# XuyangBai/D3Feat

Measured on AMD Instinct MI355X. Metric: fragments/sec (30k-pt clouds), higher is better.
Workload: dtype f32; 1 GPU; SURVEY §8d config #2: synthetic 3DMatch room fragment, 300k raw pts -> grid subsample 0.03 m (~29k pts per cloud) -> self-pair -> 5-level pyramid -> full KPFCNN forward (random-init weights (reference initialiser, seed 42), 14.1M params)...; points_per_cloud=29369, fragments_per_gpu=2141, parallelism=fragment-dp1, fragments_per_replay=12, engine_fallbacks=0, engine_isolated_replays=0

## Files before the change

### d3feat_amd/csrc/grid_subsample.hip

```cpp
#include <cstdlib>
#include "prims.h"
#include "radix_sort.h"

#define GS_EMPTY 0xFFFFFFFFFFFFFFFFull
#define GS_KEYBITS 56
#define GS_KEYMASK ((1ull << GS_KEYBITS) - 1ull)
#define GS_MAX_PROBE 4096

__constant__ unsigned long long D3F_CHAIN_DEV[D3F_NCHAIN] = {
    13ull, 29ull, 59ull, 127ull, 257ull, 541ull, 1109ull, 2357ull, 5087ull, 10273ull, 20753ull, 42043ull, 85229ull,
    172933ull, 351061ull, 712697ull, 1447153ull, 2938679ull, 5967347ull, 12117689ull, 24607243ull, 49969847ull,
    101473717ull, 206062531ull, 418451333ull, 849749479ull, 1725587117ull, 3504151727ull};

struct GsElem {
    float org[3];
    int pad0;
    unsigned long long NX, NY, NZ;
    long long bbase;
};

#include "gs_order.h"

__device__ __forceinline__ float gs_axis(unsigned mn, unsigned mx, float dl, float inv, float& org) {
    org = __fmul_rn(floorf(__fmul_rn(d3f_ord2f(mn), inv)), dl);
    return fmaxf(floorf(__fdiv_rn(__fsub_rn(d3f_ord2f(mx), org), dl)), 0.f);
}
__device__ __forceinline__ int gs_cell(const float* __restrict__ p, float ox, float oy, float oz, float dl, float& cx, float& cy,
                                       float& cz) {
    const float fx = floorf(__fdiv_rn(__fsub_rn(p[0], ox), dl));
    const float fy = floorf(__fdiv_rn(__fsub_rn(p[1], oy), dl));
    const float fz = floorf(__fdiv_rn(__fsub_rn(p[2], oz), dl));
    cx = fmaxf(fx, 0.f);
    cy = fmaxf(fy, 0.f);
    cz = fmaxf(fz, 0.f);
    return (fx < 0.f || fy < 0.f || fz < 0.f) ? D3F_ST_NEG_CELL : 0;
}

__device__ __forceinline__ float gs_inv_count(int c) { return (float)(1.0 / (double)c); }

__device__ __forceinline__ unsigned long long gs_mix(unsigned long long x) {
    x ^= x >> 33; x *= 0xff51afd7ed558ccdull; x ^= x >> 33; x *= 0xc4ceb9fe1a85ec53ull; x ^= x >> 33;
    return x;
}

__device__ __forceinline__ int gs_bits(unsigned long long x) {
    int b = 0;
    while (x) { ++b; x >>= 1; }
    return b;
}
__device__ __forceinline__ void gs_prep(const unsigned* __restrict__ bbox, const int* __restrict__ offs, int B, float dl,
                                        GsElem* __restrict__ el, int* __restrict__ status, RsMeta* __restrict__ smeta,
                                        int n_cap) {
    __shared__ unsigned long long sCells[256];
    const int b = threadIdx.x;
    unsigned long long cells = 0ull;
    if (b < B) {
        GsElem e;
        e.pad0 = 0;
        const int len = offs[b + 1] - offs[b];
        if (len <= 0) {
            atomicOr(&status[1], D3F_ST_EMPTY_ELEMENT);
            e.org[0] = e.org[1] = e.org[2] = 0.f;
            e.NX = e.NY = e.NZ = 1;
        } else {
            const float inv = __fdiv_rn(1.0f, dl);
            unsigned long long dims[3];
#pragma unroll
            for (int d = 0; d < 3; ++d) {
                const unsigned mn = __hip_atomic_load(&bbox[b * 6 + d], __ATOMIC_RELAXED, __HIP_MEMORY_SCOPE_AGENT);
                const unsigned mx = __hip_atomic_load(&bbox[b * 6 + 3 + d], __ATOMIC_RELAXED, __HIP_MEMORY_SCOPE_AGENT);
                dims[d] = (unsigned long long)gs_axis(mn, mx, dl, inv, e.org[d]) + 1ull;
            }
            e.NX = dims[0]; e.NY = dims[1]; e.NZ = dims[2];
        }
        long long base = 0;
        for (int j = 0; j < b; ++j) {
            long long l = offs[j + 1] - offs[j];
            unsigned long long nb = D3F_CHAIN_DEV[D3F_NCHAIN - 1];
            for (int c = 0; c < D3F_NCHAIN; ++c)
                if ((long long)D3F_CHAIN_DEV[c] >= l) { nb = D3F_CHAIN_DEV[c]; break; }
            base += (long long)nb;
        }
        e.bbase = base;
        el[b] = e;
        const double c = (double)e.NX * (double)e.NY * (double)e.NZ;
        cells = c >= 1.8e19 ? 0xFFFFFFFFFFFFFFFFull : e.NX * e.NY * e.NZ;
    }
    if (!smeta) return;
    sCells[threadIdx.x] = cells;
    __syncthreads();
    if (threadIdx.x == 0) {
        unsigned long long mx = 1ull;
        for (int j = 0; j < B; ++j) mx = sCells[j] > mx ? sCells[j] : mx;
        int kb = gs_bits(mx - 1ull);
        if (kb < 1) kb = 1;
        const int eb = gs_bits((unsigned long long)(B - 1));
        RsMeta m;
        m.n = min(offs[B], n_cap);
        m.kb = kb;
        m.bits = kb + eb;
        if (m.bits > 32) {
            atomicOr(&status[1], D3F_ST_KEY_WIDTH);
            m.n = 0;
            m.bits = 8;
        }
        m.npass = (m.bits + 7) / 8;
        *smeta = m;
    }
}
struct GsPrepEpi {
    const unsigned* bbox; const int* offs; int B; float dl; GsElem* el; int* status; RsMeta* smeta; int n_cap;
    __device__ __forceinline__ void operator()() const { gs_prep(bbox, offs, B, dl, el, status, smeta, n_cap); }
};

__global__ void __launch_bounds__(256) gs_begin_boxed_kernel(const int* __restrict__ lens, int B, int* __restrict__ offs,
                                                             const unsigned* __restrict__ bbox, unsigned* __restrict__ counters,
                                                             int ncounters, D3fFill f0, D3fFill fmeta, float dl, GsElem* __restrict__ el,
                                                             int* __restrict__ status, RsMeta* __restrict__ smeta, int n_cap) {
    const size_t tid = (size_t)blockIdx.x * blockDim.x + threadIdx.x, stride = (size_t)gridDim.x * blockDim.x;
    d3f_fill_words(f0, tid, stride);
    if (blockIdx.x != 0) return;
    if (threadIdx.x == 0) {
        int s = 0;
        for (int b = 0; b < B; ++b) { offs[b] = s; s += lens[b]; }
        offs[B] = s;
    }
    for (int i = threadIdx.x; i < ncounters; i += blockDim.x) counters[i] = 0u;
    for (int i = threadIdx.x; i < (int)fmeta.n; i += blockDim.x) fmeta.p[i] = fmeta.v;
    asm volatile("s_waitcnt vmcnt(0)" ::: "memory");
    __syncthreads();
    gs_prep(bbox, offs, B, dl, el, status, smeta, n_cap);
}

__global__ void __launch_bounds__(256) gs_insert_kernel(const float* __restrict__ pts, int N, const int* __restrict__ offs,
                                                        int B, float dl, const GsElem* __restrict__ el,
                                                        unsigned long long* __restrict__ tkey, unsigned* __restrict__ tfirst,
                                                        unsigned long long capmask, int* __restrict__ slot,
                                                        int* __restrict__ status) {
    const int i = blockIdx.x * blockDim.x + threadIdx.x;
    if (i >= min(N, offs[B])) return;
    const int b = d3f_find_elem(offs, B, i);
    const GsElem e = el[b];
    float cx, cy, cz;
    int st = gs_cell(pts + 3 * (size_t)i, e.org[0], e.org[1], e.org[2], dl, cx, cy, cz);
    const unsigned long long ix = (unsigned long long)cx, iy = (unsigned long long)cy, iz = (unsigned long long)cz;
    const unsigned long long key = ix + e.NX * iy + e.NX * e.NY * iz;
    if (key > GS_KEYMASK) st |= D3F_ST_KEY_RANGE;
    if (st) atomicOr(&status[1], st);
    const unsigned long long word = ((unsigned long long)b << GS_KEYBITS) | (key & GS_KEYMASK);
    unsigned long long h = gs_mix(word) & capmask;
    bool placed = false;
    for (int probe = 0; probe < GS_MAX_PROBE; ++probe) {
        unsigned long long prev = atomicCAS(&tkey[h], GS_EMPTY, word);
        if (prev == GS_EMPTY || prev == word) { placed = true; break; }
        h = (h + 1) & capmask;
    }
    if (!placed) atomicOr(&status[1], D3F_ST_OUT_OVERFLOW);
    atomicMin(&tfirst[h], (unsigned)i);
    slot[i] = (int)h;
}

struct GsMarkIn {
    const int* n_dev; const int* slot; const unsigned* tfirst;
    __device__ __forceinline__ int operator()(int i) const { return (i < *n_dev && tfirst[slot[i]] == (unsigned)i) ? 1 : 0; }
// ... 262 lines not shown
    }
    __syncthreads();
    const int w = threadIdx.x >> 6, lane = threadIdx.x & 63;
    const int base = tile * RS_TILE + w * RS_WAVE_ITEMS + lane;
    const int wlo = tile * RS_TILE + w * RS_WAVE_ITEMS, whi = min(wlo + RS_WAVE_ITEMS, n) - 1;
    int b0 = 0;
    while (b0 + 1 < B && wlo >= sOffs[b0 + 1]) ++b0;
    const bool one_cloud = (b0 + 1 >= B) || whi < sOffs[b0 + 1];
    unsigned key[RS_ROUNDS], vm = 0u;
    int st = 0;
#pragma unroll
    for (int r = 0; r < RS_ROUNDS; ++r) {
        const int i = base + r * 64;
        key[r] = 0u;
        if (i < n) {
            int b = b0;
            if (!one_cloud)
                while (b + 1 < B && i >= sOffs[b + 1]) ++b;
            const float ox = sEl[b].org[0], oy = sEl[b].org[1], oz = sEl[b].org[2];
            const unsigned NX = (unsigned)sEl[b].NX, NY = (unsigned)sEl[b].NY;
            const float* __restrict__ P = sBase[b];
            float cx, cy, cz;
            st |= gs_cell(P + 3 * (size_t)i, ox, oy, oz, dl, cx, cy, cz);
            const unsigned ix = (unsigned)cx, iy = (unsigned)cy, iz = (unsigned)cz;
            const unsigned k = ix + NX * (iy + NY * iz);
            key[r] = (kb < 32 ? ((unsigned)b << kb) : 0u) | (kb < 32 ? (k & ((1u << kb) - 1u)) : k);
            skey[i] = key[r];
            vm |= 1u << r;
        }
    }
    if (st) atomicOr(&status[1], st);
    rs_tile_histogram(key, vm, 0, sHist, hist + (size_t)tile * 256);
}

__global__ void __launch_bounds__(256) gs_heads_kernel(int N, const RsMeta* __restrict__ smeta, const unsigned* __restrict__ key0,
                                                       const unsigned* __restrict__ key1, const unsigned* __restrict__ val0,
                                                       const unsigned* __restrict__ val1, unsigned* __restrict__ fbits) {
    const int j = blockIdx.x * blockDim.x + threadIdx.x;
    if (j >= min(N, smeta->n)) return;
    const unsigned* __restrict__ ks = (smeta->npass & 1) ? key1 : key0;
    const unsigned* __restrict__ vs = (smeta->npass & 1) ? val1 : val0;
    const unsigned k = ks[j];
    if (j == 0 || ks[j - 1] != k) {
        const unsigned i = vs[j];
        atomicOr(&fbits[i >> 5], 1u << (i & 31u));
    }
}
struct GsBitsIn {
    const unsigned* fbits;
    __device__ __forceinline__ int operator()(int w) const { return __popc(fbits[w]); }
};
__global__ void __launch_bounds__(256) gs_runs_kernel(int N, const RsMeta* __restrict__ smeta, const unsigned* __restrict__ key0,
                                                      const unsigned* __restrict__ key1, const unsigned* __restrict__ val0,
                                                      const unsigned* __restrict__ val1, GsRankBits rank,
                                                      const float* __restrict__ pts, const float* const* __restrict__ ptrs,
                                                      const int* __restrict__ offs, unsigned long long* __restrict__ vkey,
                                                      float* __restrict__ bary) {
    __shared__ float sx[256], sy[256], sz[256];
    __shared__ unsigned sk[256];
    const int n = min(N, smeta->n);
    const int j0 = blockIdx.x * 256;
    if (j0 >= n) return;
    const int t = threadIdx.x, j = j0 + t;
    const unsigned* __restrict__ ks = (smeta->npass & 1) ? key1 : key0;
    const unsigned* __restrict__ vs = (smeta->npass & 1) ? val1 : val0;
    unsigned k = 0u, pi = 0u, kprev = 0u;
    float px = 0.f, py = 0.f, pz = 0.f;
    if (j < n) {
        k = ks[j];
        pi = vs[j];
        kprev = j > 0 ? ks[j - 1] : 0u;
        if (ptrs) {
            const int b = smeta->kb < 32 ? (int)(k >> smeta->kb) : 0;
            pts = ptrs[b] - 3 * (size_t)offs[b];
        }
        px = pts[3 * (size_t)pi + 0]; py = pts[3 * (size_t)pi + 1]; pz = pts[3 * (size_t)pi + 2];
    }
    sx[t] = px; sy[t] = py; sz[t] = pz;
    sk[t] = k;
    __syncthreads();
    if (j >= n || (j != 0 && kprev == k)) return;
    const int v = rank((int)pi);
    float ax = px, ay = py, az = pz;
    int c = 1;
    const int lim = min(256, n - j0);
    while (t + c < lim && sk[t + c] == k) {
        ax = __fadd_rn(ax, sx[t + c]);
        ay = __fadd_rn(ay, sy[t + c]);
        az = __fadd_rn(az, sz[t + c]);
        ++c;
    }
    if (t + c == 256) {
        while (j + c < n && ks[j + c] == k) {
            const size_t q = vs[j + c];
            ax = __fadd_rn(ax, pts[3 * q + 0]);
            ay = __fadd_rn(ay, pts[3 * q + 1]);
            az = __fadd_rn(az, pts[3 * q + 2]);
            ++c;
        }
    }
    const float sc = gs_inv_count(c);
    vkey[v] = (unsigned long long)(smeta->kb < 32 ? (k & ((1u << smeta->kb) - 1u)) : k);
    bary[3 * (size_t)v + 0] = __fmul_rn(ax, sc);
    bary[3 * (size_t)v + 1] = __fmul_rn(ay, sc);
    bary[3 * (size_t)v + 2] = __fmul_rn(az, sc);
}
template <bool BOX>
__global__ void __launch_bounds__(BOX ? 1024 : 256) gs_emit_kernel(int* __restrict__ status, const int* __restrict__ moffs, int B,
                                                      const int* __restrict__ vpos, const float* __restrict__ bary,
                                                      float* __restrict__ out_p, int out_cap, unsigned* __restrict__ bbox_out) {
    const int v = blockIdx.x * blockDim.x + threadIdx.x;
    bool ok = v < status[0] && !(status[1] & (D3F_ST_OUT_OVERFLOW | D3F_ST_KEY_WIDTH));
    int b = -1;
    float x = 0.f, y = 0.f, z = 0.f;
    if (ok) {
        b = d3f_find_elem(moffs, B, v);
        const size_t dest = (size_t)moffs[b] + (size_t)vpos[v];
        if (dest >= (size_t)out_cap) {
            atomicOr(&status[1], D3F_ST_OUT_OVERFLOW);
            ok = false;
        } else {
            x = bary[3 * (size_t)v + 0]; y = bary[3 * (size_t)v + 1]; z = bary[3 * (size_t)v + 2];
            out_p[3 * dest + 0] = x;
            out_p[3 * dest + 1] = y;
            out_p[3 * dest + 2] = z;
        }
// ... 49 lines not shown
    const size_t dest = (size_t)moffs[b] + (size_t)vpos[v];
    for (int l = 0; l < ldim; ++l) atomicMax(&out_c[dest * ldim + l], cls[(size_t)i * ldim + l]);
}

struct GsLayout {
    size_t cap;
    long long bucket_total;
};
static GsLayout gs_layout(int N, int B, int keys = -1) {
    GsLayout L;
    L.cap = 64;
    const size_t nk = (size_t)((keys > 0 && keys < N) ? keys : (N > 0 ? N : 1));
    while (L.cap < (size_t)2 * nk) L.cap <<= 1;
    L.bucket_total = (long long)(2.24 * (double)N) + 16ll * B + 64;
    return L;
}

extern "C" size_t d3f_grid_subsample_workspace_bytes(int N, int B, int fdim, int ldim) {
    (void)fdim; (void)ldim;
    if (N < 0 || B < 1) return 0;
    GsLayout L = gs_layout(N, B);
    size_t n = (size_t)(N > 0 ? N : 1);
    size_t bytes = 0;
    bytes += d3f_align((B + 1) * sizeof(int)) * 2 + d3f_align((B + 2) * sizeof(int));
    bytes += d3f_align(B * 6 * sizeof(unsigned));
    bytes += d3f_align(B * sizeof(GsElem));
    bytes += d3f_align(L.cap * sizeof(unsigned long long));
    bytes += d3f_align(L.cap * sizeof(int));
    bytes += d3f_align(n * sizeof(unsigned long long));
    bytes += 16 * d3f_align(n * sizeof(int));
    bytes += 6 * d3f_align((size_t)L.bucket_total * sizeof(int));
    bytes += d3f_align((n / GS_TILE + B + 8) * sizeof(int));
    bytes += 2 * d3f_align(d3f_scan_base_ints(N) * sizeof(int)) + d3f_align((4 + D3F_NCHAIN * (size_t)B) * sizeof(unsigned));
    bytes += d3f_align(rs_hist_words(N) * sizeof(unsigned)) + d3f_align((n / 32 + 2) * sizeof(unsigned)) +
             d3f_align(3 * n * sizeof(float)) + d3f_align(sizeof(RsMeta));
    bytes += d3f_align(7 * (size_t)B * (n < 16384 ? n : 16384) * sizeof(float)) + 256 + 2 * d3f_align(B * sizeof(int));
    return bytes + 4096;
}

template <int T, int R>
static int gs_small_launch(const GsSmallArgs& A, float* sub_points, int* sub_lens_dev, int* status_dev, hipStream_t stream) {
    static std::atomic<unsigned long long> lds_done{0ull};
    const void* const fns[] = {(const void*)gs_small_kernel<T, R>};
    if (d3f_opt_in_lds(lds_done, fns, (int)gss_lds_bytes<T, R>(GSS_NB_MAX)) != D3F_OK) return D3F_ERR_HIP;
    gs_small_kernel<T, R><<<A.B, T, gss_lds_bytes<T, R>(A.nbmax), stream>>>(A);
    D3F_LAUNCH_CHECK();
    gs_small_pack_kernel<<<d3f_cdiv(A.out_cap, 256), 256, 0, stream>>>(A, sub_points, sub_lens_dev, status_dev);
    D3F_LAUNCH_CHECK();
    return D3F_OK;
}
static int gs_run_small(const float* points, int N, const int* lens_dev, int B, float dl, float* sub_points, int M_cap, int elem_cap,
                        int pc, int* sub_lens_dev, int* status_dev, void* workspace, size_t workspace_bytes, hipStream_t stream,
                        unsigned* bbox_out = nullptr) {
    if (elem_cap <= 0 || elem_cap > M_cap) elem_cap = M_cap;
    if (elem_cap > pc) elem_cap = pc;
    D3fArena ar(workspace, workspace_bytes);
    GsSmallArgs A;
    A.stage = ar.take<float>(3 * (size_t)B * (size_t)elem_cap);
    A.recs = ar.take<float>(4 * (size_t)B * (size_t)elem_cap);
    A.mcount = ar.take<int>(B);
    A.cflags = ar.take<int>(B);
    if (!ar.ok) return D3F_ERR_WORKSPACE;
    A.bbox_out = bbox_out;
    A.pts = points; A.lens = lens_dev; A.B = B; A.dl = dl; A.elem_cap = elem_cap; A.pc = pc; A.out_cap = M_cap;
    A.nbmax = GSS_NB_MAX;
    for (int j = 0; j < D3F_NCHAIN; ++j)
        if ((long long)D3F_CHAIN_HOST[j] >= (long long)elem_cap) { A.nbmax = (int)D3F_CHAIN_HOST[j]; break; }
    if (A.nbmax > GSS_NB_MAX) A.nbmax = GSS_NB_MAX;
// ... 8 lines not shown
struct GsCall {
    const float* points; int N; const int* lens_dev; int B; float dl;
    const float* features; int fdim; const int* classes; int ldim;
    float* sub_points; int M_cap; float* sub_features; int* sub_classes; int* sub_lens_dev;
    int* status_host;
    int* status_dev;
    hipStream_t stream;
    const float* const* ptrs;
    const unsigned* bbox_in;
    unsigned* bbox_out;
};

struct GsWork {
    GsLayout L;
    int *offs, *moffs;
    unsigned* bbox;
    GsElem* el;
    int ncounters;
    unsigned* counters;
    unsigned long long* tkey;
    unsigned* tfirst;
    int* vhead;
    int* meta;
    int* vcnt;
    unsigned long long* vkey;
    int *slot, *vscan, *pvid, *pnext, *vstart, *sorted;
    GsOrderArgs A;
    int* vbase;
    int* sbase;
    unsigned* rs_hist;
    unsigned* fbits;
    float* bary;
    RsMeta* smeta;

    bool carve(void* workspace, size_t workspace_bytes, int N, int B, int keys) {
        L = gs_layout(N, B, keys);
        D3fArena ar(workspace, workspace_bytes);
        const size_t n = (size_t)N;
        offs = ar.take<int>(B + 1);
        moffs = ar.take<int>(B + 1);
        bbox = ar.take<unsigned>(B * 6);
        el = ar.take<GsElem>(B);
        ncounters = 4 + D3F_NCHAIN * B;
        counters = ar.take<unsigned>(ncounters);
        tkey = ar.take<unsigned long long>(L.cap);
        tfirst = ar.take<unsigned>(L.cap);
        vhead = ar.take<int>(n);
        meta = ar.take<int>(B + 2);
        vcnt = ar.take<int>(n);
        vkey = ar.take<unsigned long long>(n);
        slot = ar.take<int>(n);
        vscan = ar.take<int>(n);
        pvid = ar.take<int>(n);
        pnext = ar.take<int>(n);
        vstart = ar.take<int>(n);
        sorted = ar.take<int>(n);
        A.vpos = ar.take<int>(n);
        A.P[0] = ar.take<int>(n);
        A.P[1] = ar.take<int>(n);
        A.nx[0] = ar.take<int>(n);
        A.nx[1] = ar.take<int>(n);
        A.cd = ar.take<int>(n);
        A.bkt[0] = ar.take<int>(n);
        A.bkt[1] = ar.take<int>(n);
        for (int k = 0; k < 2; ++k) {
            A.bf[k] = ar.take<int>((size_t)L.bucket_total);
            A.bc[k] = ar.take<int>((size_t)L.bucket_total);
            A.bh[k] = ar.take<int>((size_t)L.bucket_total);
        }
        A.tsum = ar.take<int>(n / GS_TILE + B + 8);
        vbase = ar.take<int>(d3f_scan_base_ints(N));
        sbase = ar.take<int>(d3f_scan_base_ints(N));
        rs_hist = ar.take<unsigned>(rs_hist_words(N));
        fbits = ar.take<unsigned>(n / 32 + 2);
        bary = ar.take<float>(3 * n);
        smeta = ar.take<RsMeta>(1);
        A.vkey = vkey; A.moffs = moffs; A.offs = offs; A.el = el;
        return ar.ok;
    }
};

static int gs_order_launch(const GsWork& W, int B, int maxM, hipStream_t stream) {
    gs_order_small_kernel<<<B, GS_SMALL_T, 0, stream>>>(W.A);
    for (int j = GS_SMALL_LAST + 1; j < D3F_NCHAIN && (long long)D3F_CHAIN_HOST[j - 1] < (long long)maxM; ++j) {
        const long long nbj = (long long)D3F_CHAIN_HOST[j];
        const int hi = (int)((long long)maxM < nbj ? (long long)maxM : nbj);
        const bool more = j + 1 < D3F_NCHAIN && nbj < (long long)maxM;
        const long long nbn = more ? (long long)D3F_CHAIN_HOST[j + 1] : 0;
        const int hin = more ? (int)((long long)maxM < nbn ? (long long)maxM : nbn) : hi;
        dim3 g(d3f_cdiv(hi, 256), B), gt(d3f_cdiv(hi, GS_TILE), B), gp(d3f_cdiv(hin > hi ? hin : hi, 256), B);
        if (j == GS_SMALL_LAST + 1) gs_order_insert_kernel<<<g, 256, 0, stream>>>(W.A, j);
        gs_order_scan_tiles_kernel<<<gt, 256, 0, stream>>>(W.A, j, B, W.counters + 4 + j * B);
        gs_order_place_kernel<<<gp, 256, 0, stream>>>(W.A, j);
    }
    D3F_LAUNCH_CHECK();
    return D3F_OK;
}

static int gs_run_sort(const GsCall& C, const GsWork& W, int elem_cap) {
    const int N = C.N, B = C.B;
    const size_t n = (size_t)N;
    hipStream_t stream = C.stream;
    int rc;
    const D3fFill none{nullptr, 0ull, 0u};
    const D3fFill fill_bits{W.fbits, (unsigned long long)(n / 32 + 2), 0u};
    const D3fFill fill_meta{(unsigned*)W.meta, (unsigned long long)(B + 2), 0u};
    if (C.bbox_in) {
        long long blocks = (long long)(fill_bits.n / 4 / 256) + 1;
        if (blocks > 1024) blocks = 1024;
        gs_begin_boxed_kernel<<<(int)blocks, 256, 0, stream>>>(C.lens_dev, B, W.offs, C.bbox_in, W.counters, W.ncounters, fill_bits,
                                                               fill_meta, C.dl, W.el, W.meta, W.smeta, N);
        D3F_LAUNCH_CHECK();
    } else {
        if ((rc = d3f_begin_launch(C.lens_dev, B, W.offs, W.bbox, W.counters, W.ncounters, fill_bits, fill_meta, none, none,
                                   stream)) != D3F_OK)
            return rc;
        GsPrepEpi prep{W.bbox, W.offs, B, C.dl, W.el, W.meta, W.smeta, N};
        if ((rc = d3f_bbox_launch_t(C.points, W.offs, B, N, W.bbox, W.counters, prep, stream, C.ptrs)) != D3F_OK) return rc;
    }
    const int nblk = d3f_cdiv(N, 256);
    unsigned *key0 = (unsigned*)W.slot, *key1 = (unsigned*)W.pnext, *val0 = (unsigned*)W.pvid, *val1 = (unsigned*)W.sorted;
    gs_sortkey_kernel<<<rs_tiles(N), RS_THREADS, 0, stream>>>(C.points, C.ptrs, W.offs, B, C.dl, W.el, W.smeta, key0, W.rs_hist,
                                                              W.meta);
    D3F_LAUNCH_CHECK();
    if ((rc = rs_sort_launch(W.smeta, N, key0, key1, val0, val1, W.rs_hist, stream)) != D3F_OK) return rc;
    gs_heads_kernel<<<nblk, 256, 0, stream>>>(N, W.smeta, key0, key1, val0, val1, W.fbits);
    D3F_LAUNCH_CHECK();
    const GsRankBits rank{W.fbits, W.vscan, W.vbase};
    GsMoffsEpi<GsRankBits> mepi{W.offs, B, rank, W.meta, W.moffs, C.sub_lens_dev, C.status_dev, C.M_cap, elem_cap};
    if ((rc = d3f_scan_fold_launch(GsBitsIn{W.fbits}, N / 32 + 1, nullptr, W.vscan, W.vbase, W.counters + 1, mepi, stream)) != D3F_OK)
        return rc;
    gs_runs_kernel<<<nblk, 256, 0, stream>>>(N, W.smeta, key0, key1, val0, val1, rank, C.points, C.ptrs, W.offs, W.vkey, W.bary);
    D3F_LAUNCH_CHECK();
    const int M = N < C.M_cap ? N : C.M_cap;
    if ((rc = gs_order_launch(W, B, elem_cap, stream)) != D3F_OK) return rc;
    if (C.bbox_out)
        gs_emit_kernel<true><<<d3f_cdiv(M, 1024), 1024, 0, stream>>>(W.meta, W.moffs, B, W.A.vpos, W.bary, C.sub_points, C.M_cap,
                                                                     C.bbox_out);
    else
        gs_emit_kernel<false><<<d3f_cdiv(M, 256), 256, 0, stream>>>(W.meta, W.moffs, B, W.A.vpos, W.bary, C.sub_points, C.M_cap,
                                                                    nullptr);
    D3F_LAUNCH_CHECK();
    return D3F_OK;
}

static int gs_run_hash(const GsCall& C, const GsWork& W, int elem_cap) {
    const int N = C.N, B = C.B;
    const size_t n = (size_t)N;
    const bool async = C.status_dev != nullptr;
    hipStream_t stream = C.stream;
    int rc;
    const D3fFill none{nullptr, 0ull, 0u};
    const unsigned long long ones_words = (unsigned long long)((char*)(W.vhead + n) - (char*)W.tkey) / 4ull;
    const unsigned long long zero_words = (unsigned long long)((char*)(W.vcnt + n) - (char*)W.meta) / 4ull;
    if ((rc = d3f_begin_launch(C.lens_dev, B, W.offs, W.bbox, W.counters, W.ncounters, D3fFill{(unsigned*)W.tkey, ones_words, 0xFFFFFFFFu},
                               D3fFill{(unsigned*)W.meta, zero_words, 0u}, none, none, stream)) != D3F_OK)
        return rc;
    GsPrepEpi prep{W.bbox, W.offs, B, C.dl, W.el, W.meta, nullptr, N};
    if ((rc = d3f_bbox_launch_t(C.points, W.offs, B, N, W.bbox, W.counters, prep, stream, C.ptrs)) != D3F_OK) return rc;
    const int nblk = d3f_cdiv(N, 256);
    GsMoffsEpi<GsRankScan> mepi{W.offs, B, GsRankScan{W.vscan, W.vbase}, W.meta, W.moffs, C.sub_lens_dev, C.status_dev, C.M_cap,
                                async ? elem_cap : 0x7fffffff};
    gs_insert_kernel<<<nblk, 256, 0, stream>>>(C.points, N, W.offs, B, C.dl, W.el, W.tkey, W.tfirst, (unsigned long long)W.L.cap - 1ull,
                                               W.slot, W.meta);
    D3F_LAUNCH_CHECK();
    if ((rc = d3f_scan_fold_launch(GsMarkIn{W.offs + B, W.slot, W.tfirst}, N, W.offs + B, W.vscan, W.vbase, W.counters + 1, mepi,
                                   stream)) != D3F_OK)
        return rc;
    int M, maxM;
    if (!async) {
        D3F_HIP_TRY(hipMemcpyAsync(C.status_host, W.meta, (B + 2) * sizeof(int), hipMemcpyDeviceToHost, stream));
        D3F_HIP_TRY(hipStreamSynchronize(stream));
        M = C.status_host[0];
        if (C.status_host[1] != 0 || M <= 0) return D3F_OK;
        maxM = 0;
        for (int b = 0; b < B; ++b) maxM = C.status_host[2 + b] > maxM ? C.status_host[2 + b] : maxM;
    } else {
        M = N < C.M_cap ? N : C.M_cap;
        maxM = elem_cap;
    }
    gs_chain_kernel<<<nblk, 256, 0, stream>>>(N, W.slot, W.tfirst, W.tkey, W.vscan, W.vbase, W.pvid, W.vkey, W.vhead, W.vcnt, W.pnext,
                                              W.offs + B);
    D3F_LAUNCH_CHECK();
    if ((rc = d3f_scan_fold_launch(D3fScanIn{W.vcnt}, async ? N : M, W.meta, W.vstart, W.sbase, W.counters + 2, D3fNoEpi{},
                                   stream)) != D3F_OK)
        return rc;
    gs_rank_kernel<<<nblk, 256, 0, stream>>>(N, W.offs + B, W.pvid, W.vhead, W.pnext, W.vstart, W.sbase, W.sorted);
    if ((rc = gs_order_launch(W, B, maxM, stream)) != D3F_OK) return rc;
    gs_accum_kernel<<<d3f_cdiv(async ? N : M, 256), 256, 0, stream>>>(C.points, C.features, C.fdim, W.meta, W.moffs, B, W.vstart,
                                                                     W.sbase, W.vcnt, W.sorted, W.A.vpos, C.sub_points,
                                                                     C.sub_features, C.M_cap);
// ... 117 lines not shown
```

### d3feat_amd/csrc/radix_sort.h

```cpp
#pragma once
#include "common.h"

#define RS_THREADS 512
#define RS_WAVES (RS_THREADS / 64)
#define RS_ROUNDS 16
#define RS_TILE (RS_THREADS * RS_ROUNDS)
#define RS_WAVE_ITEMS (64 * RS_ROUNDS)
#define RS_MAX_PASSES 4

struct RsMeta {
    int n;
    int bits;
    int npass;
    int kb;
};

#define RS_SCATTER_LDS_BYTES ((2 * RS_WAVES * 256 + 256 + 16 + 2 * RS_TILE) * 4)
static inline int rs_tiles(int n_cap) { return d3f_cdiv(n_cap > 0 ? n_cap : 1, RS_TILE); }
static inline size_t rs_hist_words(int n_cap) { return (size_t)rs_tiles(n_cap) * 256; }

#ifdef __HIPCC__
__device__ __forceinline__ void rs_tile_histogram(const unsigned (&key)[RS_ROUNDS], unsigned valid_mask, int shift,
                                                  unsigned* __restrict__ sHist, unsigned* __restrict__ hist_row) {
    if (threadIdx.x < 256) sHist[threadIdx.x] = 0u;
    __syncthreads();
#pragma unroll
    for (int r = 0; r < RS_ROUNDS; ++r)
        if (valid_mask & (1u << r)) atomicAdd(&sHist[(key[r] >> shift) & 255u], 1u);
    __syncthreads();
    if (threadIdx.x < 256) hist_row[threadIdx.x] = sHist[threadIdx.x];
}

template <int W>
__device__ __forceinline__ unsigned rs_wave_bases(unsigned (*sCnt)[256], unsigned* sScan) {
    const int tid = threadIdx.x, w = tid >> 6;
    unsigned cnt = 0u;
    if (tid < 256) {
#pragma unroll
        for (int q = 0; q < W; ++q) cnt += sCnt[q][tid];
    }
    const unsigned x = d3f_wave_incl_scan(cnt);
    if ((tid & 63) == 63) sScan[w] = x;
    __syncthreads();
    unsigned loc = 0u;
    if (tid < 256) {
        unsigned wb = 0u;
#pragma unroll
        for (int q = 0; q < 4; ++q) wb += (q < w) ? sScan[q] : 0u;
        loc = wb + x - cnt;
        unsigned run = loc;
#pragma unroll
        for (int q = 0; q < W; ++q) {
            const unsigned c = sCnt[q][tid];
            sCnt[q][tid] = run;
            run += c;
        }
    }
    return loc;
}

__global__ void __launch_bounds__(RS_THREADS) rs_hist_kernel(const RsMeta* __restrict__ meta, int pass,
                                                             const unsigned* __restrict__ key0,
                                                             const unsigned* __restrict__ key1,
// ... 113 lines not shown
            __builtin_amdgcn_wave_barrier();
            if (below == 0u) myCnt[dg] = prev + (unsigned)__popcll(peers);
        }
        __builtin_amdgcn_wave_barrier();
    }
    __syncthreads();
    {
        const unsigned loc = rs_wave_bases<RS_WAVES>(sCnt, sScan);
        if (tid < 256) sBase[tid] -= loc;
    }
    __syncthreads();
#pragma unroll
    for (int r = 0; r < RS_ROUNDS; ++r) {
        if ((base + r * 64) < n) {
            const unsigned dg = (key[r] >> shift) & 255u;
            const unsigned pl = myCnt[dg] + rank[r];
            sKey[pl] = key[r];
            sVal[pl] = val[r];
        }
    }
    __syncthreads();
    const int tile_n = min(RS_TILE, n - tile * RS_TILE);
#pragma unroll
    for (int r = 0; r < RS_ROUNDS; ++r) {
        const int pl = r * RS_THREADS + tid;
        if (pl < tile_n) {
            const unsigned k = sKey[pl];
            const unsigned dest = sBase[(k >> shift) & 255u] + (unsigned)pl;
            kdst[dest] = k;
            vdst[dest] = sVal[pl];
        }
    }
}
#endif

static inline int rs_sort_launch(const RsMeta* meta, int n_cap, unsigned* key0, unsigned* key1, unsigned* val0, unsigned* val1,
                                 unsigned* hist, hipStream_t stream) {
    const int tiles = rs_tiles(n_cap);
    static std::atomic<unsigned long long> lds_done{0ull};
    const void* const fns[] = {(const void*)rs_scatter_kernel};
    if (d3f_opt_in_lds(lds_done, fns, RS_SCATTER_LDS_BYTES) != D3F_OK) return D3F_ERR_HIP;
    for (int p = 0; p < RS_MAX_PASSES; ++p) {
        if (p > 0) {
            rs_hist_kernel<<<tiles, RS_THREADS, 0, stream>>>(meta, p, key0, key1, hist);
            D3F_LAUNCH_CHECK();
        }
        rs_scatter_kernel<<<tiles, RS_THREADS, RS_SCATTER_LDS_BYTES, stream>>>(meta, p, key0, key1, val0, val1, hist);
        D3F_LAUNCH_CHECK();
    }
    return D3F_OK;
}
```

Baseline: 2002 fragments/s.

## Sort grid-subsample keys per cloud segment with 9-bit radix digits

Replaces the global radix sort over (cloud id | cell key) with a segmented radix sort. Each cloud's points are sorted only within their own offset range using 9-bit digits, so the cloud-id bits drop out of the key and fewer passes are needed. Head detection and run accumulation are adapted to treat segment boundaries as run starts. The cost is extra per-segment tiles, larger histograms and LDS, and boundary lookups in the heads and runs kernels; the old path stays available via an environment variable.

```diff
diff --git a/d3feat_amd/csrc/grid_subsample.hip b/d3feat_amd/csrc/grid_subsample.hip
--- a/d3feat_amd/csrc/grid_subsample.hip
+++ b/d3feat_amd/csrc/grid_subsample.hip
@@ -50,7 +50,7 @@
 }
 __device__ __forceinline__ void gs_prep(const unsigned* __restrict__ bbox, const int* __restrict__ offs, int B, float dl,
                                         GsElem* __restrict__ el, int* __restrict__ status, RsMeta* __restrict__ smeta,
-                                        int n_cap) {
+                                        int n_cap, int* __restrict__ tile_first) {
     __shared__ unsigned long long sCells[256];
     const int b = threadIdx.x;
     unsigned long long cells = 0ull;
@@ -105,18 +105,24 @@
             m.bits = 8;
         }
         m.npass = (m.bits + 7) / 8;
+        if (tile_first) {
+            if (m.n > 0) m.bits = kb;
+            m.npass = (m.bits + RS_SEG_BITS - 1) / RS_SEG_BITS;
+            rs_seg_tile_first(offs, B, m.n, tile_first);
+        }
         *smeta = m;
     }
 }
 struct GsPrepEpi {
-    const unsigned* bbox; const int* offs; int B; float dl; GsElem* el; int* status; RsMeta* smeta; int n_cap;
-    __device__ __forceinline__ void operator()() const { gs_prep(bbox, offs, B, dl, el, status, smeta, n_cap); }
+    const unsigned* bbox; const int* offs; int B; float dl; GsElem* el; int* status; RsMeta* smeta; int n_cap; int* tile_first;
+    __device__ __forceinline__ void operator()() const { gs_prep(bbox, offs, B, dl, el, status, smeta, n_cap, tile_first); }
 };
 
 __global__ void __launch_bounds__(256) gs_begin_boxed_kernel(const int* __restrict__ lens, int B, int* __restrict__ offs,
                                                              const unsigned* __restrict__ bbox, unsigned* __restrict__ counters,
                                                              int ncounters, D3fFill f0, D3fFill fmeta, float dl, GsElem* __restrict__ el,
-                                                             int* __restrict__ status, RsMeta* __restrict__ smeta, int n_cap) {
+                                                             int* __restrict__ status, RsMeta* __restrict__ smeta, int n_cap,
+                                                             int* __restrict__ tile_first) {
     const size_t tid = (size_t)blockIdx.x * blockDim.x + threadIdx.x, stride = (size_t)gridDim.x * blockDim.x;
     d3f_fill_words(f0, tid, stride);
     if (blockIdx.x != 0) return;
@@ -129,7 +135,7 @@
     for (int i = threadIdx.x; i < (int)fmeta.n; i += blockDim.x) fmeta.p[i] = fmeta.v;
     asm volatile("s_waitcnt vmcnt(0)" ::: "memory");
     __syncthreads();
-    gs_prep(bbox, offs, B, dl, el, status, smeta, n_cap);
+    gs_prep(bbox, offs, B, dl, el, status, smeta, n_cap, tile_first);
 }
 
 __global__ void __launch_bounds__(256) gs_insert_kernel(const float* __restrict__ pts, int N, const int* __restrict__ offs,
@@ -458,16 +464,59 @@
     if (st) atomicOr(&status[1], st);
     rs_tile_histogram(key, vm, 0, sHist, hist + (size_t)tile * 256);
 }
-
+__global__ void __launch_bounds__(RS_THREADS) gs_sortkey_seg_kernel(const float* __restrict__ pts, const float* const* __restrict__ ptrs,
+                                                                    const int* __restrict__ offs, const int* __restrict__ tile_first,
+                                                                    int B, float dl, const GsElem* __restrict__ el,
+                                                                    const RsMeta* __restrict__ smeta, unsigned* __restrict__ skey,
+                                                                    unsigned* __restrict__ hist, int* __restrict__ status) {
+    __shared__ unsigned sHist[RS_SEG_DIGITS];
+    RsSeg S;
+    if (!rs_seg_of_tile(offs, tile_first, B, smeta->n, blockIdx.x, S)) return;
+    const int b = S.e;
+    const float ox = el[b].org[0], oy = el[b].org[1], oz = el[b].org[2];
+    const unsigned NX = (unsigned)el[b].NX, NY = (unsigned)el[b].NY;
+    const float* __restrict__ P = ptrs ? ptrs[b] - 3 * (size_t)offs[b] : pts;
+    const int w = threadIdx.x >> 6, lane = threadIdx.x & 63;
+    const int base = S.first + S.lo + w * RS_WAVE_ITEMS + lane, end = S.first + S.len;
+    unsigned key[RS_ROUNDS], vm = 0u;
+    int st = 0;
+#pragma unroll
+    for (int r = 0; r < RS_ROUNDS; ++r) {
+        const int i = base + r * 64;
+        key[r] = 0u;
+        if (i < end) {
+            float cx, cy, cz;
+            st |= gs_cell(P + 3 * (size_t)i, ox, oy, oz, dl, cx, cy, cz);
+            key[r] = (unsigned)cx + NX * ((unsigned)cy + NY * (unsigned)cz);
+            skey[i] = key[r];
+            vm |= 1u << r;
+        }
+    }
+    if (st) atomicOr(&status[1], st);
+    rs_tile_histogram<RS_SEG_BITS>(key, vm, 0, sHist, hist + (size_t)blockIdx.x * RS_SEG_DIGITS);
+}
+
+__device__ __forceinline__ int gs_elem_from(const int* __restrict__ offs, int B, int b0, int j) {
+    int b = b0;
+    while (b + 1 < B && j >= offs[b + 1]) ++b;
+    return b;
+}
+
+template <bool SEG>
 __global__ void __launch_bounds__(256) gs_heads_kernel(int N, const RsMeta* __restrict__ smeta, const unsigned* __restrict__ key0,
                                                        const unsigned* __restrict__ key1, const unsigned* __restrict__ val0,
-                                                       const unsigned* __restrict__ val1, unsigned* __restrict__ fbits) {
+                                                       const unsigned* __restrict__ val1, unsigned* __restrict__ fbits,
+                                                       const int* __restrict__ offs, int B) {
     const int j = blockIdx.x * blockDim.x + threadIdx.x;
     if (j >= min(N, smeta->n)) return;
     const unsigned* __restrict__ ks = (smeta->npass & 1) ? key1 : key0;
     const unsigned* __restrict__ vs = (smeta->npass & 1) ? val1 : val0;
     const unsigned k = ks[j];
-    if (j == 0 || ks[j - 1] != k) {
+    bool head = j == 0 || ks[j - 1] != k;
+    if constexpr (SEG) {
+        if (!head) head = j == offs[gs_elem_from(offs, B, d3f_find_elem(offs, B, blockIdx.x * blockDim.x), j)];
+    }
+    if (head) {
         const unsigned i = vs[j];
         atomicOr(&fbits[i >> 5], 1u << (i & 31u));
     }
@@ -476,12 +525,13 @@
     const unsigned* fbits;
     __device__ __forceinline__ int operator()(int w) const { return __popc(fbits[w]); }
 };
+template <bool SEG>
 __global__ void __launch_bounds__(256) gs_runs_kernel(int N, const RsMeta* __restrict__ smeta, const unsigned* __restrict__ key0,
                                                       const unsigned* __restrict__ key1, const unsigned* __restrict__ val0,
                                                       const unsigned* __restrict__ val1, GsRankBits rank,
                                                       const float* __restrict__ pts, const float* const* __restrict__ ptrs,
-                                                      const int* __restrict__ offs, unsigned long long* __restrict__ vkey,
-                                                      float* __restrict__ bary) {
+                                                      const int* __restrict__ offs, int B,
+                                                      unsigned long long* __restrict__ vkey, float* __restrict__ bary) {
     __shared__ float sx[256], sy[256], sz[256];
     __shared__ unsigned sk[256];
     const int n = min(N, smeta->n);
@@ -492,24 +542,31 @@
     const unsigned* __restrict__ vs = (smeta->npass & 1) ? val1 : val0;
     unsigned k = 0u, pi = 0u, kprev = 0u;
     float px = 0.f, py = 0.f, pz = 0.f;
+    int end = n;
+    bool first = false;
     if (j < n) {
         k = ks[j];
         pi = vs[j];
         kprev = j > 0 ? ks[j - 1] : 0u;
-        if (ptrs) {
-            const int b = smeta->kb < 32 ? (int)(k >> smeta->kb) : 0;
-            pts = ptrs[b] - 3 * (size_t)offs[b];
-        }
+        int b;
+        if constexpr (SEG) {
+            b = gs_elem_from(offs, B, d3f_find_elem(offs, B, j0), j);
+            first = j == offs[b];
+            end = min(offs[b + 1], n);
+        } else {
+            b = smeta->kb < 32 ? (int)(k >> smeta->kb) : 0;
+        }
+        if (ptrs) pts = ptrs[b] - 3 * (size_t)offs[b];
         px = pts[3 * (size_t)pi + 0]; py = pts[3 * (size_t)pi + 1]; pz = pts[3 * (size_t)pi + 2];
     }
     sx[t] = px; sy[t] = py; sz[t] = pz;
     sk[t] = k;
     __syncthreads();
-    if (j >= n || (j != 0 && kprev == k)) return;
+    if (j >= n || (j != 0 && kprev == k && !first)) return;
     const int v = rank((int)pi);
     float ax = px, ay = py, az = pz;
     int c = 1;
-    const int lim = min(256, n - j0);
+    const int lim = min(256, end - j0);
     while (t + c < lim && sk[t + c] == k) {
         ax = __fadd_rn(ax, sx[t + c]);
         ay = __fadd_rn(ay, sy[t + c]);
@@ -517,7 +574,7 @@
         ++c;
     }
     if (t + c == 256) {
-        while (j + c < n && ks[j + c] == k) {
+        while (j + c < end && ks[j + c] == k) {
             const size_t q = vs[j + c];
             ax = __fadd_rn(ax, pts[3 * q + 0]);
             ay = __fadd_rn(ay, pts[3 * q + 1]);
@@ -633,8 +690,8 @@
     bytes += 6 * d3f_align((size_t)L.bucket_total * sizeof(int));
     bytes += d3f_align((n / GS_TILE + B + 8) * sizeof(int));
     bytes += 2 * d3f_align(d3f_scan_base_ints(N) * sizeof(int)) + d3f_align((4 + D3F_NCHAIN * (size_t)B) * sizeof(unsigned));
-    bytes += d3f_align(rs_hist_words(N) * sizeof(unsigned)) + d3f_align((n / 32 + 2) * sizeof(unsigned)) +
-             d3f_align(3 * n * sizeof(float)) + d3f_align(sizeof(RsMeta));
+    bytes += d3f_align(rs_seg_hist_words(N, B) * sizeof(unsigned)) + d3f_align((n / 32 + 2) * sizeof(unsigned)) +
+             d3f_align(3 * n * sizeof(float)) + d3f_align(sizeof(RsMeta)) + d3f_align((B + 1) * sizeof(int));
     bytes += d3f_align(7 * (size_t)B * (n < 16384 ? n : 16384) * sizeof(float)) + 256 + 2 * d3f_align(B * sizeof(int));
     return bytes + 4096;
 }
@@ -709,6 +766,7 @@
     unsigned* fbits;
     float* bary;
     RsMeta* smeta;
+    int* tile_first;
 
     bool carve(void* workspace, size_t workspace_bytes, int N, int B, int keys) {
         L = gs_layout(N, B, keys);
@@ -748,10 +806,11 @@
         A.tsum = ar.take<int>(n / GS_TILE + B + 8);
         vbase = ar.take<int>(d3f_scan_base_ints(N));
         sbase = ar.take<int>(d3f_scan_base_ints(N));
-        rs_hist = ar.take<unsigned>(rs_hist_words(N));
+        rs_hist = ar.take<unsigned>(rs_seg_hist_words(N, B));
         fbits = ar.take<unsigned>(n / 32 + 2);
         bary = ar.take<float>(3 * n);
         smeta = ar.take<RsMeta>(1);
+        tile_first = ar.take<int>(B + 1);
         A.vkey = vkey; A.moffs = moffs; A.offs = offs; A.el = el;
         return ar.ok;
     }
@@ -775,6 +834,11 @@
 }
 
 static int gs_run_sort(const GsCall& C, const GsWork& W, int elem_cap) {
+    static const bool seg = [] {
+        const char* e = getenv("D3F_GS_SEGSORT");
+        return !(e && e[0] == '0' && e[1] == 0);
+    }();
+    int* const tile_first = seg ? W.tile_first : nullptr;
     const int N = C.N, B = C.B;
     const size_t n = (size_t)N;
     hipStream_t stream = C.stream;
@@ -786,28 +850,41 @@
         long long blocks = (long long)(fill_bits.n / 4 / 256) + 1;
         if (blocks > 1024) blocks = 1024;
         gs_begin_boxed_kernel<<<(int)blocks, 256, 0, stream>>>(C.lens_dev, B, W.offs, C.bbox_in, W.counters, W.ncounters, fill_bits,
-                                                               fill_meta, C.dl, W.el, W.meta, W.smeta, N);
+                                                               fill_meta, C.dl, W.el, W.meta, W.smeta, N, tile_first);
         D3F_LAUNCH_CHECK();
     } else {
         if ((rc = d3f_begin_launch(C.lens_dev, B, W.offs, W.bbox, W.counters, W.ncounters, fill_bits, fill_meta, none, none,
                                    stream)) != D3F_OK)
             return rc;
-        GsPrepEpi prep{W.bbox, W.offs, B, C.dl, W.el, W.meta, W.smeta, N};
+        GsPrepEpi prep{W.bbox, W.offs, B, C.dl, W.el, W.meta, W.smeta, N, tile_first};
         if ((rc = d3f_bbox_launch_t(C.points, W.offs, B, N, W.bbox, W.counters, prep, stream, C.ptrs)) != D3F_OK) return rc;
     }
     const int nblk = d3f_cdiv(N, 256);
     unsigned *key0 = (unsigned*)W.slot, *key1 = (unsigned*)W.pnext, *val0 = (unsigned*)W.pvid, *val1 = (unsigned*)W.sorted;
-    gs_sortkey_kernel<<<rs_tiles(N), RS_THREADS, 0, stream>>>(C.points, C.ptrs, W.offs, B, C.dl, W.el, W.smeta, key0, W.rs_hist,
-                                                              W.meta);
-    D3F_LAUNCH_CHECK();
-    if ((rc = rs_sort_launch(W.smeta, N, key0, key1, val0, val1, W.rs_hist, stream)) != D3F_OK) return rc;
-    gs_heads_kernel<<<nblk, 256, 0, stream>>>(N, W.smeta, key0, key1, val0, val1, W.fbits);
+    if (seg) {
+        gs_sortkey_seg_kernel<<<rs_seg_tiles(N, B), RS_THREADS, 0, stream>>>(C.points, C.ptrs, W.offs, tile_first, B, C.dl, W.el, W.smeta,
+                                                                            key0, W.rs_hist, W.meta);
+        D3F_LAUNCH_CHECK();
+        if ((rc = rs_seg_sort_launch(W.smeta, W.offs, tile_first, B, N, key0, key1, val0, val1, W.rs_hist, stream)) != D3F_OK) return rc;
+        gs_heads_kernel<true><<<nblk, 256, 0, stream>>>(N, W.smeta, key0, key1, val0, val1, W.fbits, W.offs, B);
+    } else {
+        gs_sortkey_kernel<<<rs_tiles(N), RS_THREADS, 0, stream>>>(C.points, C.ptrs, W.offs, B, C.dl, W.el, W.smeta, key0, W.rs_hist,
+                                                                  W.meta);
+        D3F_LAUNCH_CHECK();
+        if ((rc = rs_sort_launch(W.smeta, N, key0, key1, val0, val1, W.rs_hist, stream)) != D3F_OK) return rc;
+        gs_heads_kernel<false><<<nblk, 256, 0, stream>>>(N, W.smeta, key0, key1, val0, val1, W.fbits, W.offs, B);
+    }
     D3F_LAUNCH_CHECK();
     const GsRankBits rank{W.fbits, W.vscan, W.vbase};
     GsMoffsEpi<GsRankBits> mepi{W.offs, B, rank, W.meta, W.moffs, C.sub_lens_dev, C.status_dev, C.M_cap, elem_cap};
     if ((rc = d3f_scan_fold_launch(GsBitsIn{W.fbits}, N / 32 + 1, nullptr, W.vscan, W.vbase, W.counters + 1, mepi, stream)) != D3F_OK)
         return rc;
-    gs_runs_kernel<<<nblk, 256, 0, stream>>>(N, W.smeta, key0, key1, val0, val1, rank, C.points, C.ptrs, W.offs, W.vkey, W.bary);
+    if (seg)
+        gs_runs_kernel<true><<<nblk, 256, 0, stream>>>(N, W.smeta, key0, key1, val0, val1, rank, C.points, C.ptrs, W.offs, B, W.vkey,
+                                                       W.bary);
+    else
+        gs_runs_kernel<false><<<nblk, 256, 0, stream>>>(N, W.smeta, key0, key1, val0, val1, rank, C.points, C.ptrs, W.offs, B, W.vkey,
+                                                        W.bary);
     D3F_LAUNCH_CHECK();
     const int M = N < C.M_cap ? N : C.M_cap;
     if ((rc = gs_order_launch(W, B, elem_cap, stream)) != D3F_OK) return rc;
@@ -833,7 +910,7 @@
     if ((rc = d3f_begin_launch(C.lens_dev, B, W.offs, W.bbox, W.counters, W.ncounters, D3fFill{(unsigned*)W.tkey, ones_words, 0xFFFFFFFFu},
                                D3fFill{(unsigned*)W.meta, zero_words, 0u}, none, none, stream)) != D3F_OK)
         return rc;
-    GsPrepEpi prep{W.bbox, W.offs, B, C.dl, W.el, W.meta, nullptr, N};
+    GsPrepEpi prep{W.bbox, W.offs, B, C.dl, W.el, W.meta, nullptr, N, nullptr};
     if ((rc = d3f_bbox_launch_t(C.points, W.offs, B, N, W.bbox, W.counters, prep, stream, C.ptrs)) != D3F_OK) return rc;
     const int nblk = d3f_cdiv(N, 256);
     GsMoffsEpi<GsRankScan> mepi{W.offs, B, GsRankScan{W.vscan, W.vbase}, W.meta, W.moffs, C.sub_lens_dev, C.status_dev, C.M_cap,
diff --git a/d3feat_amd/csrc/radix_sort.h b/d3feat_amd/csrc/radix_sort.h
--- a/d3feat_amd/csrc/radix_sort.h
+++ b/d3feat_amd/csrc/radix_sort.h
@@ -19,16 +19,24 @@
 static inline int rs_tiles(int n_cap) { return d3f_cdiv(n_cap > 0 ? n_cap : 1, RS_TILE); }
 static inline size_t rs_hist_words(int n_cap) { return (size_t)rs_tiles(n_cap) * 256; }
 
+#define RS_SEG_BITS 9
+#define RS_SEG_DIGITS (1 << RS_SEG_BITS)
+#define RS_SEG_SCATTER_LDS_BYTES ((2 * RS_WAVES * RS_SEG_DIGITS + RS_SEG_DIGITS + 16 + 2 * RS_TILE) * 4)
+static inline int rs_seg_tiles(int n_cap, int B) { return rs_tiles(n_cap) + B; }
+static inline size_t rs_seg_hist_words(int n_cap, int B) { return (size_t)rs_seg_tiles(n_cap, B) * RS_SEG_DIGITS; }
+
 #ifdef __HIPCC__
+template <int BITS = 8>
 __device__ __forceinline__ void rs_tile_histogram(const unsigned (&key)[RS_ROUNDS], unsigned valid_mask, int shift,
                                                   unsigned* __restrict__ sHist, unsigned* __restrict__ hist_row) {
-    if (threadIdx.x < 256) sHist[threadIdx.x] = 0u;
+    static_assert((1 << BITS) <= RS_THREADS, "one thread per bin");
+    if (threadIdx.x < (1 << BITS)) sHist[threadIdx.x] = 0u;
     __syncthreads();
 #pragma unroll
     for (int r = 0; r < RS_ROUNDS; ++r)
-        if (valid_mask & (1u << r)) atomicAdd(&sHist[(key[r] >> shift) & 255u], 1u);
-    __syncthreads();
-    if (threadIdx.x < 256) hist_row[threadIdx.x] = sHist[threadIdx.x];
+        if (valid_mask & (1u << r)) atomicAdd(&sHist[(key[r] >> shift) & ((1u << BITS) - 1u)], 1u);
+    __syncthreads();
+    if (threadIdx.x < (1 << BITS)) hist_row[threadIdx.x] = sHist[threadIdx.x];
 }
 
 template <int W>
@@ -208,6 +216,209 @@
         }
     }
 }
+
+__device__ __forceinline__ int rs_seg_len(const int* __restrict__ offs, int e, int n, int& first) {
+    first = max(min(offs[e], n), 0);
+    return max(min(offs[e + 1], n), first) - first;
+}
+__device__ __forceinline__ void rs_seg_tile_first(const int* __restrict__ offs, int B, int n, int* __restrict__ tile_first) {
+    int t = 0, first;
+    for (int e = 0; e < B; ++e) {
+        tile_first[e] = t;
+        t += (rs_seg_len(offs, e, n, first) + RS_TILE - 1) / RS_TILE;
+    }
+    tile_first[B] = t;
+}
+struct RsSeg {
+    int e;
+    int first;
+    int len;
+    int lo;
+    int row0;
+    int rows;
+};
+__device__ __forceinline__ bool rs_seg_of_tile(const int* __restrict__ offs, const int* __restrict__ tile_first, int B, int n,
+                                               int tile, RsSeg& s) {
+    if (tile >= tile_first[B]) return false;
+    const int e = d3f_find_elem(tile_first, B, tile);
+    s.e = e;
+    s.len = rs_seg_len(offs, e, n, s.first);
+    s.row0 = tile_first[e];
+    s.rows = tile_first[e + 1] - s.row0;
+    s.lo = (tile - s.row0) * RS_TILE;
+    return true;
+}
+
+static_assert(RS_THREADS == RS_SEG_DIGITS, "one thread per digit");
+__device__ __forceinline__ unsigned rs_seg_wave_bases(unsigned (*sCnt)[RS_SEG_DIGITS], unsigned* sScan) {
+    const int tid = threadIdx.x, w = tid >> 6;
+    unsigned cnt = 0u;
+#pragma unroll
+    for (int q = 0; q < RS_WAVES; ++q) cnt += sCnt[q][tid];
+    const unsigned x = d3f_wave_incl_scan(cnt);
+    if ((tid & 63) == 63) sScan[w] = x;
+    __syncthreads();
+    unsigned wb = 0u;
+#pragma unroll
+    for (int q = 0; q < RS_WAVES; ++q) wb += (q < w) ? sScan[q] : 0u;
+    const unsigned loc = wb + x - cnt;
+    unsigned run = loc;
+#pragma unroll
+    for (int q = 0; q < RS_WAVES; ++q) {
+        const unsigned c = sCnt[q][tid];
+        sCnt[q][tid] = run;
+        run += c;
+    }
+    return loc;
+}
+
+__global__ void __launch_bounds__(RS_THREADS) rs_seg_hist_kernel(const RsMeta* __restrict__ meta, int pass,
+                                                                 const int* __restrict__ offs, const int* __restrict__ tile_first,
+                                                                 int B, const unsigned* __restrict__ key0,
+                                                                 const unsigned* __restrict__ key1, unsigned* __restrict__ hist) {
+    __shared__ unsigned sHist[RS_SEG_DIGITS];
+    if (pass >= meta->npass) return;
+    RsSeg S;
+    if (!rs_seg_of_tile(offs, tile_first, B, meta->n, blockIdx.x, S)) return;
+    const unsigned* __restrict__ src = ((pass & 1) ? key1 : key0) + S.first;
+    const int w = threadIdx.x >> 6, lane = threadIdx.x & 63;
+    const int base = S.lo + w * RS_WAVE_ITEMS + lane;
+    unsigned key[RS_ROUNDS], vm = 0u;
+#pragma unroll
+    for (int r = 0; r < RS_ROUNDS; ++r) {
+        const int pos = base + r * 64;
+        key[r] = 0u;
+        if (pos < S.len) { key[r] = src[pos]; vm |= 1u << r; }
+    }
+    rs_tile_histogram<RS_SEG_BITS>(key, vm, pass * RS_SEG_BITS, sHist, hist + (size_t)blockIdx.x * RS_SEG_DIGITS);
+}
+
+__global__ void __launch_bounds__(RS_THREADS) rs_seg_scatter_kernel(const RsMeta* __restrict__ meta, int pass,
+                                                                    const int* __restrict__ offs,
+                                                                    const int* __restrict__ tile_first, int B,
+                                                                    unsigned* __restrict__ key0, unsigned* __restrict__ key1,
+                                                                    unsigned* __restrict__ val0, unsigned* __restrict__ val1,
+                                                                    const unsigned* __restrict__ hist) {
+    extern __shared__ __attribute__((aligned(16))) unsigned rs_seg_lds[];
+    unsigned (*sCnt)[RS_SEG_DIGITS] = (unsigned (*)[RS_SEG_DIGITS])rs_seg_lds;
+    unsigned (*sPart)[RS_SEG_DIGITS] = (unsigned (*)[RS_SEG_DIGITS])(rs_seg_lds + RS_WAVES * RS_SEG_DIGITS);
+    unsigned* sBase = rs_seg_lds + 2 * RS_WAVES * RS_SEG_DIGITS;
+    unsigned* sScan = sBase + RS_SEG_DIGITS;
+    unsigned* sKey = sScan + 16;
+    unsigned* sVal = sKey + RS_TILE;
+    if (pass >= meta->npass) return;
+    RsSeg S;
+    if (!rs_seg_of_tile(offs, tile_first, B, meta->n, blockIdx.x, S)) return;
+    const unsigned* __restrict__ ksrc = ((pass & 1) ? key1 : key0) + S.first;
+    const unsigned* __restrict__ vsrc = ((pass & 1) ? val1 : val0) + S.first;
+    unsigned* __restrict__ kdst = (pass & 1) ? key0 : key1;
+    unsigned* __restrict__ vdst = (pass & 1) ? val0 : val1;
+    const int tid = threadIdx.x, w = tid >> 6, lane = tid & 63;
+    const int shift = pass * RS_SEG_BITS;
+
+    const int base = S.lo + w * RS_WAVE_ITEMS + lane;
+    unsigned key[RS_ROUNDS], val[RS_ROUNDS];
+#pragma unroll
+    for (int r = 0; r < RS_ROUNDS; ++r) {
+        const int pos = base + r * 64;
+        key[r] = 0u;
+        val[r] = (unsigned)(S.first + pos);
+        if (pos < S.len) {
+            key[r] = ksrc[pos];
+            if (pass > 0) val[r] = vsrc[pos];
+        }
+    }
+    {
+        uint4 bef = make_uint4(0u, 0u, 0u, 0u), tot = make_uint4(0u, 0u, 0u, 0u);
+        const int mine = (int)blockIdx.x - S.row0;
+        const uint4* __restrict__ rows = (const uint4*)(hist + (size_t)S.row0 * RS_SEG_DIGITS) + (w & 1) * 64 + lane;
+        int t = w >> 1;
+        for (; t + 12 < S.rows; t += 16) {
+            uint4 v[4];
+#pragma unroll
+            for (int u = 0; u < 4; ++u) v[u] = rows[(size_t)(t + 4 * u) * (RS_SEG_DIGITS / 4)];
+#pragma unroll
+            for (int u = 0; u < 4; ++u) {
+                tot.x += v[u].x; tot.y += v[u].y; tot.z += v[u].z; tot.w += v[u].w;
+                if (t + 4 * u < mine) { bef.x += v[u].x; bef.y += v[u].y; bef.z += v[u].z; bef.w += v[u].w; }
+            }
+        }
+        for (; t < S.rows; t += 4) {
+            const uint4 v = rows[(size_t)t * (RS_SEG_DIGITS / 4)];
+            tot.x += v.x; tot.y += v.y; tot.z += v.z; tot.w += v.w;
+            if (t < mine) { bef.x += v.x; bef.y += v.y; bef.z += v.z; bef.w += v.w; }
+        }
+        ((uint4*)sCnt[w])[lane] = tot;
+        ((uint4*)sPart[w])[lane] = bef;
+    }
+    __syncthreads();
+    {
+        unsigned total = 0u, before = 0u;
+        const int half = tid >> 8, c = tid & 255;
+#pragma unroll
+        for (int q = 0; q < RS_WAVES / 2; ++q) { total += sCnt[2 * q + half][c]; before += sPart[2 * q + half][c]; }
+        const unsigned x = d3f_wave_incl_scan(total);
+        if (lane == 63) sScan[w] = x;
+        __syncthreads();
+#pragma unroll
+        for (int q = 0; q < RS_WAVES; ++q) sCnt[q][tid] = 0u;
+        unsigned wb = 0u;
+#pragma unroll
+        for (int q = 0; q < RS_WAVES; ++q) wb += (q < w) ? sScan[q] : 0u;
+        sBase[tid] = (unsigned)S.first + wb + x - total + before;
+        __syncthreads();
+    }
+    unsigned rank[RS_ROUNDS];
+    volatile unsigned* myCnt = sCnt[w];
+#pragma unroll
+    for (int r = 0; r < RS_ROUNDS; ++r) {
+        const bool valid = (base + r * 64) < S.len;
+        const unsigned dg = (key[r] >> shift) & (RS_SEG_DIGITS - 1u);
+        unsigned long long peers = __ballot(valid);
+#pragma unroll
+        for (int bit = 0; bit < RS_SEG_BITS; ++bit) {
+            const bool one = (dg >> bit) & 1u;
+            const unsigned long long m = __ballot(one);
+            peers &= one ? m : ~m;
+        }
+        rank[r] = 0u;
+        if (valid) {
+            const unsigned prev = myCnt[dg];
+            const unsigned below = (unsigned)__popcll(peers & d3f_lanemask_lt());
+            rank[r] = prev + below;
+            __builtin_amdgcn_wave_barrier();
+            if (below == 0u) myCnt[dg] = prev + (unsigned)__popcll(peers);
+        }
+        __builtin_amdgcn_wave_barrier();
+    }
+    __syncthreads();
+    {
+        const unsigned loc = rs_seg_wave_bases(sCnt, sScan);
+        sBase[tid] -= loc;
+    }
+    __syncthreads();
+#pragma unroll
+    for (int r = 0; r < RS_ROUNDS; ++r) {
+        if ((base + r * 64) < S.len) {
+            const unsigned dg = (key[r] >> shift) & (RS_SEG_DIGITS - 1u);
+            const unsigned pl = myCnt[dg] + rank[r];
+            sKey[pl] = key[r];
+            sVal[pl] = val[r];
+        }
+    }
+    __syncthreads();
+    const int tile_n = min(RS_TILE, S.len - S.lo);
+#pragma unroll
+    for (int r = 0; r < RS_ROUNDS; ++r) {
+        const int pl = r * RS_THREADS + tid;
+        if (pl < tile_n) {
+            const unsigned k = sKey[pl];
+            const unsigned dest = sBase[(k >> shift) & (RS_SEG_DIGITS - 1u)] + (unsigned)pl;
+            kdst[dest] = k;
+            vdst[dest] = sVal[pl];
+        }
+    }
+}
 #endif
 
 static inline int rs_sort_launch(const RsMeta* meta, int n_cap, unsigned* key0, unsigned* key1, unsigned* val0, unsigned* val1,
@@ -226,3 +437,21 @@
     }
     return D3F_OK;
 }
+
+static inline int rs_seg_sort_launch(const RsMeta* meta, const int* offs, const int* tile_first, int B, int n_cap, unsigned* key0,
+                                     unsigned* key1, unsigned* val0, unsigned* val1, unsigned* hist, hipStream_t stream) {
+    const int tiles = rs_seg_tiles(n_cap, B);
+    static std::atomic<unsigned long long> lds_done{0ull};
+    const void* const fns[] = {(const void*)rs_seg_scatter_kernel};
+    if (d3f_opt_in_lds(lds_done, fns, RS_SEG_SCATTER_LDS_BYTES) != D3F_OK) return D3F_ERR_HIP;
+    for (int p = 0; p < RS_MAX_PASSES; ++p) {
+        if (p > 0) {
+            rs_seg_hist_kernel<<<tiles, RS_THREADS, 0, stream>>>(meta, p, offs, tile_first, B, key0, key1, hist);
+            D3F_LAUNCH_CHECK();
+        }
+        rs_seg_scatter_kernel<<<tiles, RS_THREADS, RS_SEG_SCATTER_LDS_BYTES, stream>>>(meta, p, offs, tile_first, B, key0, key1, val0,
+                                                                                       val1, hist);
+        D3F_LAUNCH_CHECK();
+    }
+    return D3F_OK;
+}
```

After: 2021 fragments/s, median of 6. About the same (+1.0%).
